# second-state/qwen3_asr_rs

Measured on NVIDIA H100. Metric: real-time factor (audio-sec/wall-sec) Qwen3-ASR-0.6B 30s clips, higher is better.
Workload: dtype f32 (bf16 weights, fp32-exact activations)

## Files before the change

qwen3_asr_rs_b200/csrc/decode_mega.cu:

```cuda
#include "mega_common.cuh"

namespace asrb {

namespace mega {

struct Params {
    const DecLayerW* layers;
    const bf16* lm_head;
    const bf16* embed;
    const float* final_norm;
    const float* rope_cos; const float* rope_sin;
    float eps;
    int L, H, QD, KVD, I, V, nq, nkv, group;
    float* x;
    float* kcache; float* vcache; size_t cache_layer_stride; int max_ctx;
    int nsplit;
    float* part_val; int* part_idx;
    int* pos; int* done; int* next_id; int* ids_out; int* n_out; int max_new;
    unsigned* bar;
    uint2* qkv_ll; uint2* part_ll; uint2* attn_ll; uint2* x_ll; uint2* act_ll;
    long long* dbg;
    int pf_ahead;
};

static constexpr int PF_AHEAD = 2;

template <int H, int QD, int I>
struct ChunkCursor {
    int l, ph, r; Slice s; bool done;
    const DecLayerW* ltab;
    __device__ void load(const Params& p) {
        if (l >= p.L) { if (l == p.L && ph == 0) s = make_slice(p.lm_head, p.V, H, 1); else { done = true; return; } }
        else {
            const DecLayerW w = ltab[l];
            s = ph == 0 ? make_slice(w.wqkv, QD + 2 * p.KVD, H, 1) : ph == 1 ? make_slice(w.wo, H, QD, 1)
              : ph == 2 ? make_slice(w.wgu, 2 * I, H, 2) : make_slice(w.wdown, H, I, 1);
        }
        r = s.r0;
    }
    __device__ void init(const Params& p, const DecLayerW* table) { ltab = table; l = 0; ph = 0; done = false; load(p); }
    __device__ bool next(const Params& p, const bf16*& src, uint32_t& bytes) {
        while (!done && r >= s.r1) {
            if (l >= p.L) { done = true; break; }
            if (++ph == 4) { ph = 0; ++l; }
            load(p);
        }
        if (done) return false;
        const int rows = min(s.rpc, s.r1 - r);
        src = s.W + (size_t)r * s.K; bytes = (uint32_t)rows * s.K * 2;
        r += s.rpc;
        return true;
    }
};

template <class Cursor>
__device__ __forceinline__ void produce(const Slice& s, const Ring& ring, uint32_t& q, Cursor& pf, const Params& p) {
    for (int r = s.r0; r < s.r1; r += s.rpc, ++q) {
        int rows = min(s.rpc, s.r1 - r);
        uint32_t slot = q % ring.nslot, par = (q / ring.nslot) & 1;
        mbar_wait(&ring.empty[slot], par ^ 1);
        uint32_t bytes = (uint32_t)rows * s.K * 2;
        mbar_expect_tx(&ring.full[slot], bytes);
        bulk_g2s(ring.slots + (size_t)slot * SLOT_BYTES, s.W + (size_t)r * s.K, bytes, &ring.full[slot]);
        const bf16* psrc; uint32_t pbytes;
        if (p.pf_ahead > 0 && pf.next(p, psrc, pbytes)) l2_prefetch(psrc, pbytes);
    }
}

template <int K>
__device__ __forceinline__ void load_xr(const float* xs, float (&xr)[K / 32], int lane) {
    const int sw = ((lane >> 2) & 1) * 4;
#pragma unroll
    for (int c = 0; c < K / 256; ++c) {
        const float4 a = *reinterpret_cast<const float4*>(xs + (c * 32 + lane) * 8 + sw);
        const float4 b = *reinterpret_cast<const float4*>(xs + (c * 32 + lane) * 8 + 4 - sw);
        xr[c * 8 + 0] = a.x; xr[c * 8 + 1] = a.y; xr[c * 8 + 2] = a.z; xr[c * 8 + 3] = a.w;
        xr[c * 8 + 4] = b.x; xr[c * 8 + 5] = b.y; xr[c * 8 + 6] = b.z; xr[c * 8 + 7] = b.w;
    }
}
template <int K>
__device__ __forceinline__ void load_xr_norm(const float* xs, const float* wn, float r, float (&xr)[K / 32], int lane) {
    const int sw = ((lane >> 2) & 1) * 4;
#pragma unroll
    for (int c = 0; c < K / 256; ++c) {
        const int o = (c * 32 + lane) * 8;
        const float4 a = *reinterpret_cast<const float4*>(xs + o + sw), b = *reinterpret_cast<const float4*>(xs + o + 4 - sw);
        const float4 wa = *reinterpret_cast<const float4*>(wn + o + sw), wb = *reinterpret_cast<const float4*>(wn + o + 4 - sw);
        xr[c * 8 + 0] = (a.x * r) * wa.x; xr[c * 8 + 1] = (a.y * r) * wa.y; xr[c * 8 + 2] = (a.z * r) * wa.z; xr[c * 8 + 3] = (a.w * r) * wa.w;
        xr[c * 8 + 4] = (b.x * r) * wb.x; xr[c * 8 + 5] = (b.y * r) * wb.y; xr[c * 8 + 6] = (b.z * r) * wb.z; xr[c * 8 + 7] = (b.w * r) * wb.w;
    }
}

template <int K>
__device__ __forceinline__ float row_dot(const uint4* wrow, const float (&xr)[K / 32], int lane) {
    float a0 = 0.f, a1 = 0.f;
#pragma unroll
    for (int c = 0; c < K / 256; ++c) {
        const uint4 w = wrow[c * 32 + lane];
        a0 = fmaf(bf16_lo(w.x), xr[c * 8 + 0], a0); a1 = fmaf(bf16_hi(w.x), xr[c * 8 + 1], a1);
        a0 = fmaf(bf16_lo(w.y), xr[c * 8 + 2], a0); a1 = fmaf(bf16_hi(w.y), xr[c * 8 + 3], a1);
        a0 = fmaf(bf16_lo(w.z), xr[c * 8 + 4], a0); a1 = fmaf(bf16_hi(w.z), xr[c * 8 + 5], a1);
        a0 = fmaf(bf16_lo(w.w), xr[c * 8 + 6], a0); a1 = fmaf(bf16_hi(w.w), xr[c * 8 + 7], a1);
    }
    return warp_sum(a0 + a1);
}
template <int K>
__device__ __forceinline__ float row_dot2(const uint4* w0, const uint4* w1, const float (&xr)[K / 32], int lane) {
    float a0 = 0.f, a1 = 0.f, b0 = 0.f, b1 = 0.f;
#pragma unroll
    for (int c = 0; c < K / 256; ++c) {
        const uint4 w = w0[c * 32 + lane], v = w1[c * 32 + lane];
        a0 = fmaf(bf16_lo(w.x), xr[c * 8 + 0], a0); a1 = fmaf(bf16_hi(w.x), xr[c * 8 + 1], a1);
        b0 = fmaf(bf16_lo(v.x), xr[c * 8 + 0], b0); b1 = fmaf(bf16_hi(v.x), xr[c * 8 + 1], b1);
        a0 = fmaf(bf16_lo(w.y), xr[c * 8 + 2], a0); a1 = fmaf(bf16_hi(w.y), xr[c * 8 + 3], a1);
        b0 = fmaf(bf16_lo(v.y), xr[c * 8 + 2], b0); b1 = fmaf(bf16_hi(v.y), xr[c * 8 + 3], b1);
        a0 = fmaf(bf16_lo(w.z), xr[c * 8 + 4], a0); a1 = fmaf(bf16_hi(w.z), xr[c * 8 + 5], a1);
        b0 = fmaf(bf16_lo(v.z), xr[c * 8 + 4], b0); b1 = fmaf(bf16_hi(v.z), xr[c * 8 + 5], b1);
        a0 = fmaf(bf16_lo(w.w), xr[c * 8 + 6], a0); a1 = fmaf(bf16_hi(w.w), xr[c * 8 + 7], a1);
        b0 = fmaf(bf16_lo(v.w), xr[c * 8 + 6], b0); b1 = fmaf(bf16_hi(v.w), xr[c * 8 + 7], b1);
    }
    const float ra = a0 + a1, rb = b0 + b1;
    const bool hi = lane & 16;
    float keep = (hi ? rb : ra) + __shfl_xor_sync(0xffffffffu, hi ? ra : rb, 16);
#pragma unroll
    for (int o = 8; o > 0; o >>= 1) keep += __shfl_xor_sync(0xffffffffu, keep, o);
    return keep;
}

template <int K>
__device__ __forceinline__ float row_dot_smem(const uint4* wrow, const float* xs, int lane) {
    float a0 = 0.f, a1 = 0.f;
    const int sw = ((lane >> 2) & 1) * 4;
#pragma unroll 4
    for (int c = 0; c < K / 256; ++c) {
        const uint4 w = wrow[c * 32 + lane];
        const float4 xa = *reinterpret_cast<const float4*>(xs + (c * 32 + lane) * 8 + sw);
        const float4 xb = *reinterpret_cast<const float4*>(xs + (c * 32 + lane) * 8 + 4 - sw);
        a0 = fmaf(bf16_lo(w.x), xa.x, a0); a1 = fmaf(bf16_hi(w.x), xa.y, a1);
        a0 = fmaf(bf16_lo(w.y), xa.z, a0); a1 = fmaf(bf16_hi(w.y), xa.w, a1);
        a0 = fmaf(bf16_lo(w.z), xb.x, a0); a1 = fmaf(bf16_hi(w.z), xb.y, a1);
        a0 = fmaf(bf16_lo(w.w), xb.z, a0); a1 = fmaf(bf16_hi(w.w), xb.w, a1);
    }
    return warp_sum(a0 + a1);
}


template <int K>
__device__ __forceinline__ float row_dot4(const uint4* w0, const uint4* w1, const uint4* w2, const uint4* w3,
                                          const float (&xr)[K / 32], int lane) {
    float a0 = 0.f, a1 = 0.f, b0 = 0.f, b1 = 0.f, c0 = 0.f, c1 = 0.f, d0 = 0.f, d1 = 0.f;
// ... 215 lines not shown
                    const bool two = ub + 1 < units_here;
                    v0 = row_dot2<KX>(base + (size_t)ub * (K / 8), base + (size_t)(two ? ub + 1 : ub) * (K / 8),
                                      reinterpret_cast<const float (&)[KX / 32]>(xr), lane);
                    act = ((lane & 15) == 0) && (sub == 0 || two);
                    row = r + ub + sub;
                } else {
                    if (XREG) v0 = row_dot<KX>(base + (size_t)ub * (K / 8), reinterpret_cast<const float (&)[KX / 32]>(xr), lane);
                    else v0 = row_dot_smem<K>(base + (size_t)ub * (K / 8), xs, lane);
                    act = lane == 0; row = r + ub;
                }
                if (EPI == ME_STORE) {
                    if (act) ll_store(out + row, v0, tag);
                } else if (EPI == ME_RESID) {
                    if (act) { const float nv = xres[row - s.r0] + v0; xres[row - s.r0] = nv; ll_store(out + row, nv, tag); }
                } else {
                    if (act && v0 > best_v) { best_v = v0; best_i = row; }
                }
            }
        }
        unit += (units_here + UPW - 1) / UPW * UPW;
        CF();
        __syncwarp();
        if (lane == 0) mbar_arrive(&ring.empty[slot]);
    }
    CF();
#undef CF
    if (!XREG) cons_sync();
}

__device__ __forceinline__ float norm_scale(float ss, int n, float eps, float* red) {
    const int tid = threadIdx.x;
    ss = warp_sum(ss);
    if ((tid & 31) == 0) red[tid >> 5] = ss;
    cons_sync();
    float tot = 0.f;
#pragma unroll
    for (int i = 0; i < NCONS_WARPS; ++i) tot += red[i];
    return 1.0f / sqrtf(tot / n + eps);
}

__device__ __forceinline__ void head_norm_rope(const uint2* __restrict__ src, uint32_t tag, const float* __restrict__ nw,
                                               float eps, const float* __restrict__ cs, const float* __restrict__ sn,
                                               float* dst, int lane) {
    float v[4];
    ll_poll4(src + lane, 32, tag, v);
    float ss = warp_sum(v[0] * v[0] + v[1] * v[1] + v[2] * v[2] + v[3] * v[3]);
    const float r = 1.0f / sqrtf(ss / 128.f + eps);
#pragma unroll
    for (int i = 0; i < 4; ++i) v[i] = (v[i] * r) * nw[lane + 32 * i];
#pragma unroll
    for (int i = 0; i < 2; ++i) {
        const int d = lane + 32 * i;
        const float c = cs[d], s = sn[d];
        const float a = v[i], b = v[i + 2];
        dst[d] = a * c - b * s;
        dst[d + 64] = b * c + a * s;
    }
}

#define MEGA_FINE(k)                                                                                    \
    do {                                                                                               \
        if (dbg_row && tid == 0 && l == 5) dbg_row[400 + (k)] = clock64();                              \
    } while (0)
#define MEGA_GT(k)                                                                                     \
    do {                                                                                               \
        if (p.dbg && tid == 0 && l == 5) {                                                             \
            unsigned long long t_; asm volatile("mov.u64 %0, %%globaltimer;" : "=l"(t_));               \
            p.dbg[512 + 3 * blockIdx.x + (k)] = (long long)t_;                                         \
        }                                                                                              \
    } while (0)
#define MEGA_MARK()                                                                                    \
    do {                                                                                               \
        if (dbg_row && tid == 0 && dbg_i < DBG_SLOTS) dbg_row[dbg_i++] = clock64();                    \
    } while (0)

template <int H, int QD, int I, int NS>
__global__ void __launch_bounds__(NTHREADS, 1) decode_step_kernel(const Params p) {
    constexpr int XS_FLOATS = (I > XS_MIN ? I : XS_MIN) + 64;
    extern __shared__ __align__(128) uint8_t smem[];
    constexpr int PARAM_FLOATS = 2 * H + 2 * HD;
    Ring ring;
    ring.slots = smem;
    ring.nslot = NS;
    uint8_t* kv_smem = smem + (size_t)NS * SLOT_BYTES;
    float* xs = reinterpret_cast<float*>(kv_smem + 2 * KV_TILE_BYTES);
    float* xres = xs + XS_FLOATS;
    float* pbuf = xres + XRES_MAX;
    float* ropes = pbuf + 2 * PARAM_FLOATS;
    DecLayerW* ltab = reinterpret_cast<DecLayerW*>(ropes + 128);
    uint64_t* bars = reinterpret_cast<uint64_t*>(ltab + MAX_LAYERS);
    ring.full = bars; ring.empty = bars + NSLOT_MAX;
    uint64_t* kv_full = bars + 2 * NSLOT_MAX; uint64_t* kv_empty = kv_full + 1;
    uint64_t* p_full = kv_empty + 1; uint64_t* p_empty = p_full + 2;
    float* red = reinterpret_cast<float*>(bars + 2 * NSLOT_MAX + 6);
    int* ired = reinterpret_cast<int*>(red + 64);
    float* part = reinterpret_cast<float*>(ired + 64);
    const int tid = threadIdx.x, lane = tid & 31, warp = tid >> 5;
    const bool is_producer = warp == NCONS_WARPS;

    if (__ldcg(p.done) != 0) return;

    if (tid == 0) {
        for (int i = 0; i < NS; ++i) { mbar_init(&ring.full[i], 1); mbar_init(&ring.empty[i], NCONS_WARPS); }
        mbar_init(kv_full, 1); mbar_init(kv_empty, NCONS_WARPS);
        for (int i = 0; i < 2; ++i) { mbar_init(&p_full[i], 1); mbar_init(&p_empty[i], NCONS_WARPS); }
        asm volatile("fence.mbarrier_init.release.cluster;" ::: "memory");
    }
    const int pos = __ldcg(p.pos);
    {
        const uint2* src = reinterpret_cast<const uint2*>(p.layers);
        uint2* dst = reinterpret_cast<uint2*>(ltab);
        for (int i = tid; i < p.L * (int)(sizeof(DecLayerW) / 8); i += NTHREADS) dst[i] = src[i];
        if (tid < 64) ropes[tid] = p.rope_cos[(size_t)pos * 64 + tid];
        else if (tid < 128) ropes[tid] = p.rope_sin[(size_t)pos * 64 + tid - 64];
    }
    __syncthreads();

    const bool att_cta = (int)blockIdx.x < p.nkv * p.nsplit;
    const int att_g = blockIdx.x / p.nsplit, att_sp = blockIdx.x % p.nsplit, att_j0 = att_sp * KV_KEYS;
    const int n_old = att_cta ? max(0, min(pos - att_j0, KV_KEYS)) : 0;
    uint32_t kvq = 0;
    uint32_t q = 0;
    if (is_producer) {
        if (lane == 0) {
            ChunkCursor<H, QD, I> pf;
            pf.init(p, ltab);
            {
                const bf16* psrc; uint32_t pbytes;
                for (int i = 0; i < p.pf_ahead; ++i) if (pf.next(p, psrc, pbytes)) l2_prefetch(psrc, pbytes);
            }
            const size_t kv_row = ((size_t)att_g * p.max_ctx + att_j0) * HD;
            if (n_old > 0) {
                l2_prefetch(p.kcache + kv_row, (uint32_t)n_old * HD * 4);
                l2_prefetch(p.vcache + kv_row, (uint32_t)n_old * HD * 4);
            }
            for (int l = 0; l <= p.L; ++l) {
                {
                    float* pb = pbuf + (l & 1) * PARAM_FLOATS;
                    mbar_wait(&p_empty[l & 1], ((l >> 1) & 1) ^ 1);
                    if (l < p.L) {
                        const DecLayerW w = ltab[l];
                        mbar_expect_tx(&p_full[l & 1], (uint32_t)(2 * H + 2 * HD) * 4);
                        bulk_g2s(pb, w.ln_in, H * 4, &p_full[l & 1]);
                        bulk_g2s(pb + H, w.ln_post, H * 4, &p_full[l & 1]);
                        bulk_g2s(pb + 2 * H, w.qnorm, HD * 4, &p_full[l & 1]);
                        bulk_g2s(pb + 2 * H + HD, w.knorm, HD * 4, &p_full[l & 1]);
                    } else {
                        mbar_expect_tx(&p_full[l & 1], (uint32_t)H * 4);
                        bulk_g2s(pb, p.final_norm, H * 4, &p_full[l & 1]);
                        break;
                    }
                }
                const DecLayerW w = ltab[l];
                produce(make_slice(w.wqkv, QD + 2 * p.KVD, H, 1), ring, q, pf, p);
                if (n_old > 0) {
                    const uint32_t bytes = (uint32_t)n_old * HD * 4;
                    if (l + 1 < p.L) {
                        l2_prefetch(p.kcache + (size_t)(l + 1) * p.cache_layer_stride + kv_row, bytes);
                        l2_prefetch(p.vcache + (size_t)(l + 1) * p.cache_layer_stride + kv_row, bytes);
                    }
                    mbar_wait(kv_empty, (kvq & 1) ^ 1);
                    mbar_expect_tx(kv_full, 2 * bytes);
                    const size_t off = (size_t)l * p.cache_layer_stride + kv_row;
                    bulk_g2s(kv_smem, p.kcache + off, bytes, kv_full);
                    bulk_g2s(kv_smem + KV_TILE_BYTES, p.vcache + off, bytes, kv_full);
                    ++kvq;
                }
                produce(make_slice(w.wo, H, QD, 1), ring, q, pf, p);
                produce(make_slice(w.wgu, 2 * I, H, 2), ring, q, pf, p);
                produce(make_slice(w.wdown, H, I, 1), ring, q, pf, p);
            }
            produce(make_slice(p.lm_head, p.V, H, 1), ring, q, pf, p);
            {
                ChunkCursor<H, QD, I> nx;
                nx.init(p, ltab);
                const bf16* psrc; uint32_t pbytes;
                for (int i = 0; i < p.pf_ahead; ++i) if (nx.next(p, psrc, pbytes)) l2_prefetch(psrc, pbytes);
            }
        }
        return;
    }

    long long* dbg_row = nullptr; int dbg_i = 0;
    if (p.dbg && (blockIdx.x == 0 || blockIdx.x == gridDim.x - 1)) dbg_row = p.dbg + (blockIdx.x == 0 ? 0 : DBG_SLOTS);
    MEGA_MARK();
    const int half = HD / 2;
    const float* cs = ropes;
    const float* sn = ropes + half;
    const unsigned G = gridDim.x;
    float best_v = -INFINITY; int best_i = 0x7fffffff;
    const unsigned epoch = __ldcg(p.bar + 1);
    const uint32_t tag_base = (epoch & 0xffffffu) << 8;
    const Slice xsl = make_slice(nullptr, H, QD, 1);
    Slice sl_qkv = make_slice(nullptr, QD + 2 * p.KVD, H, 1), sl_o = make_slice(nullptr, H, QD, 1),
          sl_gu = make_slice(nullptr, 2 * I, H, 2), sl_dn = make_slice(nullptr, H, I, 1);
    for (int i = tid; i < xsl.r1 - xsl.r0; i += NCONS) xres[i] = __ldcg(p.x + xsl.r0 + i);

    for (int l = 0; l < p.L; ++l) {
        const DecLayerW w = ltab[l];
        const uint32_t tl = tag_base | ((uint32_t)l << 3);
        const float* pb = pbuf + (l & 1) * PARAM_FLOATS;
        mbar_wait(&p_full[l & 1], (l >> 1) & 1);
        float nr;
        {
            float ss = 0.f;
            if (l == 0) { for (int i = tid; i < H; i += NCONS) { const float v = __ldcg(p.x + i); xs[xs_swz(i)] = v; ss = fmaf(v, v, ss); } }
            else { MEGA_FINE(0); MEGA_FINE(1); ss = ll_gather(p.x_ll, H, (tag_base | ((uint32_t)(l - 1) << 3)) | PH_XD, xs); MEGA_FINE(2); }
            nr = norm_scale(ss, H, p.eps, red);
            MEGA_FINE(3);
        }
        consume<H, ME_STORE>(sl_qkv, ring, q, xs, p.qkv_ll, tl | PH_QKV, xres, best_v, best_i, pb, nr);
        MEGA_FINE(4);
        MEGA_GT(0);
        MEGA_MARK();
        {
            const int nloc = n_old;
            const int nact = min(p.nsplit, (pos + KV_KEYS - 1) / KV_KEYS);
            const bool merger = att_cta && att_sp == 0;
            if (nloc > 0) {
                const int g = att_g;
                float* qs = xs;
                float* kn = qs + p.group * HD;
                float* vn = kn + HD;
                float* sc = vn + HD;
                float* ml = sc + p.group * KV_KEYS;
                float* osum = ml + 8;
                float* wml = osum + NCONS_WARPS * 2 * HD;
                float* snew = wml + NCONS_WARPS * 4;
                float* Ks = reinterpret_cast<float*>(kv_smem);
                float* Vs = reinterpret_cast<float*>(kv_smem + KV_TILE_BYTES);
                MEGA_FINE(24);
                cons_sync();
                if (warp < p.group) head_norm_rope(p.qkv_ll + (size_t)(g * p.group + warp) * HD, tl | PH_QKV, pb + 2 * H, p.eps, cs, sn, qs + warp * HD, lane);
                else if (warp == p.group && merger) head_norm_rope(p.qkv_ll + QD + (size_t)g * HD, tl | PH_QKV, pb + 2 * H + HD, p.eps, cs, sn, kn, lane);
                else if (warp == p.group + 1 && merger) {
                    float vv[4];
                    ll_poll4(p.qkv_ll + QD + p.KVD + (size_t)g * HD + lane, 32, tl | PH_QKV, vv);
#pragma unroll
                    for (int i = 0; i < 4; ++i) vn[lane + 32 * i] = vv[i];
                }
                MEGA_FINE(25);
                mbar_wait(kv_full, kvq & 1);
                cons_sync();
                MEGA_FINE(26);
                if (merger) {
                    if (tid < HD) {
                        float* kc = p.kcache + (size_t)l * p.cache_layer_stride + ((size_t)g * p.max_ctx + pos) * HD;
                        float* vc = p.vcache + (size_t)l * p.cache_layer_stride + ((size_t)g * p.max_ctx + pos) * HD;
                        kc[tid] = kn[tid]; vc[tid] = vn[tid];
                    }
                    if (warp >= NCONS_WARPS - p.group) {
                        const int hq = warp - (NCONS_WARPS - p.group);
                        const float4 a = *reinterpret_cast<const float4*>(qs + hq * HD + lane * 4);
                        const float4 b = *reinterpret_cast<const float4*>(kn + lane * 4);
                        const float sn_ = warp_sum(fmaf(a.x, b.x, fmaf(a.y, b.y, fmaf(a.z, b.z, a.w * b.w))));
                        if (lane == 0) snew[hq] = sn_ / sqrtf((float)HD);
                    }
                }
                MEGA_FINE(27);
                if (p.group == 2) {
                    const float4 q0 = *reinterpret_cast<const float4*>(qs + lane * 4);
                    const float4 q1 = *reinterpret_cast<const float4*>(qs + HD + lane * 4);
                    float pv[16];
#pragma unroll
                    for (int kk = 0; kk < 8; ++kk) {
                        const int j = warp + 8 * kk;
                        const float4 kv = *reinterpret_cast<const float4*>(Ks + j * HD + lane * 4);
                        pv[2 * kk] = fmaf(kv.x, q0.x, fmaf(kv.y, q0.y, fmaf(kv.z, q0.z, kv.w * q0.w)));
                        pv[2 * kk + 1] = fmaf(kv.x, q1.x, fmaf(kv.y, q1.y, fmaf(kv.z, q1.z, kv.w * q1.w)));
                    }
#pragma unroll
                    for (int o = 16, n = 16; n > 1; o >>= 1, n >>= 1) {
                        const bool up = lane & o;
#pragma unroll
                        for (int i = 0; i < n / 2; ++i) {
                            const float send = up ? pv[i] : pv[i + n / 2];
                            const float keep = up ? pv[i + n / 2] : pv[i];
                            pv[i] = keep + __shfl_xor_sync(0xffffffffu, send, o);
                        }
                    }
                    pv[0] += __shfl_xor_sync(0xffffffffu, pv[0], 1);
                    const bool mine = warp + 8 * (lane >> 2) < nloc;
                    const float sv = mine ? pv[0] / sqrtf((float)HD) : -INFINITY;
                    float mw = sv;
                    mw = fmaxf(mw, __shfl_xor_sync(0xffffffffu, mw, 4));
                    mw = fmaxf(mw, __shfl_xor_sync(0xffffffffu, mw, 8));
                    mw = fmaxf(mw, __shfl_xor_sync(0xffffffffu, mw, 16));
                    const float ev = mine ? expf(sv - mw) : 0.f;
                    float lw = ev;
                    lw += __shfl_xor_sync(0xffffffffu, lw, 4);
                    lw += __shfl_xor_sync(0xffffffffu, lw, 8);
                    lw += __shfl_xor_sync(0xffffffffu, lw, 16);
                    float4 o0 = make_float4(0.f, 0.f, 0.f, 0.f), o1 = o0;
#pragma unroll
                    for (int kk = 0; kk < 8; ++kk) {
                        const int j = warp + 8 * kk;
                        const float4 vv = *reinterpret_cast<const float4*>(Vs + j * HD + lane * 4);
                        const float e0 = __shfl_sync(0xffffffffu, ev, 4 * kk), e1 = __shfl_sync(0xffffffffu, ev, 4 * kk + 2);
                        if (j < nloc) {
                            o0.x = fmaf(e0, vv.x, o0.x); o0.y = fmaf(e0, vv.y, o0.y); o0.z = fmaf(e0, vv.z, o0.z); o0.w = fmaf(e0, vv.w, o0.w);
                            o1.x = fmaf(e1, vv.x, o1.x); o1.y = fmaf(e1, vv.y, o1.y); o1.z = fmaf(e1, vv.z, o1.z); o1.w = fmaf(e1, vv.w, o1.w);
                        }
                    }
                    *reinterpret_cast<float4*>(osum + (warp * 2 + 0) * HD + lane * 4) = o0;
                    *reinterpret_cast<float4*>(osum + (warp * 2 + 1) * HD + lane * 4) = o1;
                    if (lane == 0 || lane == 2) { wml[(warp * 2 + (lane >> 1)) * 2] = mw; wml[(warp * 2 + (lane >> 1)) * 2 + 1] = lw; }
                    cons_sync();
                    MEGA_FINE(28);
                    {
                        const int hq = tid / HD, d = tid - hq * HD;
                        float M = -INFINITY;
#pragma unroll
                        for (int w8 = 0; w8 < NCONS_WARPS; ++w8) M = fmaxf(M, wml[(w8 * 2 + hq) * 2]);
                        float acc = 0.f, Ls = 0.f;
#pragma unroll
                        for (int w8 = 0; w8 < NCONS_WARPS; ++w8) {
                            const float f = expf(wml[(w8 * 2 + hq) * 2] - M);
                            acc = fmaf(f, osum[(w8 * 2 + hq) * HD + d], acc);
                            Ls = fmaf(f, wml[(w8 * 2 + hq) * 2 + 1], Ls);
                        }
                        uint2* rec = p.part_ll + ((size_t)blockIdx.x * 2 + hq) * PSTRIDE;
                        ll_store(rec + d, acc, tl | PH_PART);
                        if (d < 2) ll_store(rec + HD + d, d == 0 ? M : Ls, tl | PH_PART);
                    }
                    MEGA_FINE(29);
                } else {
                    for (int idx = tid; idx < p.group * KV_KEYS; idx += NCONS) {
                        const int hq = idx / KV_KEYS, j = idx - hq * KV_KEYS;
                        if (j < nloc) {
                            const float* kr = Ks + j * HD; const float* qr = qs + hq * HD;
                            float a0 = 0.f, a1 = 0.f;
#pragma unroll 8
                            for (int dd = 0; dd < HD; dd += 2) {
                                const int d0 = (dd + j) & (HD - 1), d1 = (dd + 1 + j) & (HD - 1);
                                a0 = fmaf(kr[d0], qr[d0], a0); a1 = fmaf(kr[d1], qr[d1], a1);
                            }
                            sc[hq * KV_KEYS + j] = (a0 + a1) / sqrtf((float)HD);
                        }
                    }
                    cons_sync();
                    if (warp < p.group) {
                        float mx = -INFINITY;
                        for (int j = lane; j < nloc; j += 32) mx = fmaxf(mx, sc[warp * KV_KEYS + j]);
                        mx = warp_max(mx);
                        float sum = 0.f;
                        for (int j = lane; j < nloc; j += 32) {
                            float e = expf(sc[warp * KV_KEYS + j] - mx);
                            sc[warp * KV_KEYS + j] = e; sum += e;
                        }
                        sum = warp_sum(sum);
                        if (lane == 0) { ml[warp * 2] = mx; ml[warp * 2 + 1] = sum; }
                    }
                    cons_sync();
                    for (int idx = tid; idx < p.group * HD; idx += NCONS) {
                        const int hq = idx / HD, d = idx - hq * HD;
                        float acc = 0.f;
                        for (int j = 0; j < nloc; ++j) acc = fmaf(sc[hq * KV_KEYS + j], Vs[j * HD + d], acc);
                        uint2* rec = p.part_ll + ((size_t)blockIdx.x * p.group + hq) * PSTRIDE;
                        ll_store(rec + d, acc, tl | PH_PART);
                        if (d < 2) ll_store(rec + HD + d, ml[hq * 2 + d], tl | PH_PART);
                    }
                }
                {
                    asm volatile("fence.proxy.async.shared::cta;" ::: "memory");
                    __syncwarp();
                    if (lane == 0) mbar_arrive(kv_empty);
                    ++kvq;
                }
                MEGA_FINE(30);
                MEGA_GT(1);
                if (merger) {
                    for (int idx = tid; idx < p.group * HD; idx += NCONS) {
                        const int hq = idx / HD, d = idx - hq * HD;
                        const uint32_t tg = tl | PH_PART;
                        constexpr int RB = 9;
                        uint2 mv, lv, ov[RB];
                        bool ok;
                        auto load_round = [&](int u0) {
#pragma unroll
                            for (int u = 0; u < RB; ++u) {
                                if (u0 + u < nact) {
                                    const uint2* rec = p.part_ll + ((size_t)(g * p.nsplit + u0 + u) * p.group + hq) * PSTRIDE;
                                    asm volatile("ld.relaxed.gpu.global.v2.u32 {%0, %1}, [%2];" : "=r"(ov[u].x), "=r"(ov[u].y) : "l"(rec + d) : "memory");
                                }
                            }
                        };
                        auto round_ok = [&](int u0) {
                            bool k = true;
#pragma unroll
                            for (int u = 0; u < RB; ++u) if (u0 + u < nact) k = k && (ov[u].y == tg);
                            return k;
                        };
                        do {
                            mv.y = tg; lv.y = tg; mv.x = 0u; lv.x = 0u;
                            if (lane < nact) {
                                const uint2* rec = p.part_ll + ((size_t)(g * p.nsplit + lane) * p.group + hq) * PSTRIDE;
                                asm volatile("ld.relaxed.gpu.global.v2.u32 {%0, %1}, [%2];" : "=r"(mv.x), "=r"(mv.y) : "l"(rec + HD) : "memory");
                                asm volatile("ld.relaxed.gpu.global.v2.u32 {%0, %1}, [%2];" : "=r"(lv.x), "=r"(lv.y) : "l"(rec + HD + 1) : "memory");
                            }
                            load_round(0);
                            ok = __all_sync(0xffffffffu, (mv.y == tg) && (lv.y == tg) && round_ok(0));
                        } while (!ok);
                        MEGA_FINE(35);
                        const float m_l = lane < nact ? __uint_as_float(mv.x) : (lane == nact ? snew[hq] : -INFINITY);
                        const float l_l = lane < nact ? __uint_as_float(lv.x) : (lane == nact ? 1.f : 0.f);
                        const float M = warp_max(m_l);
                        const float f = expf(m_l - M);
                        const float Lsum = warp_sum(f * l_l);
                        float O = __shfl_sync(0xffffffffu, f, nact) * vn[d];
                        for (int u0 = 0; u0 < nact; u0 += RB) {
                            if (u0 > 0) { do { load_round(u0); ok = __all_sync(0xffffffffu, round_ok(u0)); } while (!ok); }
#pragma unroll
                            for (int u = 0; u < RB; ++u)
                                if (u0 + u < nact) O = fmaf(__shfl_sync(0xffffffffu, f, u0 + u), __uint_as_float(ov[u].x), O);
                        }
                        ll_store(p.attn_ll + (size_t)(g * p.group + hq) * HD + d, O / Lsum, tl | PH_ATTN);
                    }
                }
                MEGA_FINE(31);
                cons_sync();
            }
        }
        MEGA_MARK();
        MEGA_FINE(32);
        ll_gather(p.attn_ll, QD, tl | PH_ATTN, xs);
        MEGA_FINE(33);
        MEGA_GT(2);
        cons_sync();
        consume<QD, ME_RESID>(sl_o, ring, q, xs, p.x_ll, tl | PH_XO, xres, best_v, best_i, nullptr, 1.f, nullptr, part);
        MEGA_FINE(34);
        MEGA_MARK();
        cons_sync();
        {
            MEGA_FINE(8); MEGA_FINE(9);
            const float ss = ll_gather(p.x_ll, H, tl | PH_XO, xs); MEGA_FINE(10);
            nr = norm_scale(ss, H, p.eps, red); MEGA_FINE(11);
        }
        consume<H, ME_SWIGLU>(sl_gu, ring, q, xs, p.act_ll, tl | PH_ACT, xres, best_v, best_i, pb + H, nr, (dbg_row && l == 5) ? dbg_row + 440 : nullptr);
        MEGA_FINE(12);
        MEGA_FINE(13);
        MEGA_MARK();
        MEGA_FINE(16); MEGA_FINE(17);
        ll_gather(p.act_ll, I, tl | PH_ACT, xs); MEGA_FINE(18);
        cons_sync();
        consume<I, ME_RESID>(sl_dn, ring, q, xs, p.x_ll, tl | PH_XD, xres, best_v, best_i, nullptr, 1.f, nullptr, part);
        MEGA_FINE(19);
        MEGA_FINE(20);
        MEGA_MARK();
        cons_sync();
        if (lane == 0) mbar_arrive(&p_empty[l & 1]);
    }
    float nrf;
    {
        const float ss = ll_gather(p.x_ll, H, (tag_base | ((uint32_t)(p.L - 1) << 3)) | PH_XD, xs);
        mbar_wait(&p_full[p.L & 1], (p.L >> 1) & 1);
        nrf = norm_scale(ss, H, p.eps, red);
    }
    consume<H, ME_ARGMAX>(make_slice(p.lm_head, p.V, H, 1), ring, q, xs, nullptr, 0u, xres, best_v, best_i,
                          pbuf + (p.L & 1) * PARAM_FLOATS, nrf);
    MEGA_MARK();
#pragma unroll
    for (int o = 8; o <= 16; o <<= 1) {
        const float ov = __shfl_xor_sync(0xffffffffu, best_v, o); const int oi = __shfl_xor_sync(0xffffffffu, best_i, o);
        if (ov > best_v || (ov == best_v && oi < best_i)) { best_v = ov; best_i = oi; }
    }
    cons_sync();
    if (lane == 0) { red[warp] = best_v; ired[warp] = best_i; }
    cons_sync();
    int& is_last = ired[63];
    if (tid == 0) {
        float v = -INFINITY; int idx = 0x7fffffff;
        for (int wq = 0; wq < NCONS_WARPS; ++wq)
            if (red[wq] > v || (red[wq] == v && ired[wq] < idx)) { v = red[wq]; idx = ired[wq]; }
        p.part_val[blockIdx.x] = v; p.part_idx[blockIdx.x] = idx;
        __threadfence();
        unsigned t = atomicAdd(p.bar, 1u);
        is_last = (t == G - 1);
    }
    cons_sync();
    if (!is_last) return;
    __threadfence();
    {
        float v = -INFINITY; int idx = 0x7fffffff;
        for (int i = tid; i < (int)G; i += NCONS) {
            float pv = __ldcg(p.part_val + i); int pi = __ldcg(p.part_idx + i);
            if (pv > v || (pv == v && pi < idx)) { v = pv; idx = pi; }
        }
#pragma unroll
        for (int o = 16; o > 0; o >>= 1) {
            float ov = __shfl_xor_sync(0xffffffffu, v, o); int oi = __shfl_xor_sync(0xffffffffu, idx, o);
            if (ov > v || (ov == v && oi < idx)) { v = ov; idx = oi; }
        }
        if (lane == 0) { red[warp] = v; ired[warp] = idx; }
        cons_sync();
        int& tok_s = ired[62];
        if (tid == 0) {
            for (int wq = 1; wq < NCONS_WARPS; ++wq)
                if (red[wq] > v || (red[wq] == v && ired[wq] < idx)) { v = red[wq]; idx = ired[wq]; }
            int tok = idx;
            const int n = *p.n_out;
            if (tok == 151643 || tok == 151645 || n >= p.max_new) { *p.done = 1; *p.next_id = -1; tok = -1; }
            else { p.ids_out[n] = tok; *p.n_out = n + 1; *p.pos = pos + 1; *p.next_id = tok; }
            tok_s = tok;
            p.bar[0] = 0;
            p.bar[1] = p.bar[1] + 1;
        }
        cons_sync();
        const int tok = tok_s;
        if (tok >= 0) {
            const bf16* e = p.embed + (size_t)tok * H;
            for (int i = tid; i < H; i += NCONS) p.x[i] = __bfloat162float(e[i]);
        }
    }
}

}

static long long* g_last_dbg = nullptr;

static int mega_xs_floats(int I) { return std::max(I, mega::XS_MIN) + 64; }
static size_t mega_smem_bytes(int H, int I, int nslot) {
    return (size_t)nslot * mega::SLOT_BYTES + 2 * mega::KV_TILE_BYTES +
           (mega_xs_floats(I) + mega::XRES_MAX + 2 * (2 * H + 2 * mega::HD) + 128) * 4 + mega::MAX_LAYERS * sizeof(DecLayerW) +
           (2 * mega::NSLOT_MAX + 6) * 8 + 64 * 4 + 64 * 4 + 128 * 4 + 64;
}
static int mega_nslot(const asrb_dims& c) { return c.hidden_size > 1024 ? 3 : 4; }

template <int H, int QD, int I> static bool dims_match(const asrb_dims& c) {
    return c.hidden_size == H && c.num_attention_heads * c.head_dim == QD && c.intermediate_size == I;
}

bool decode_mega_supported(const Model& m, int B, int ctx) {
    const int max_ctx = ctx;
    const asrb_dims& c = m.d.c;
    if (B < 1 || c.head_dim != 128) return false;
    const int group = c.num_attention_heads / c.num_key_value_heads;
    if (group + 2 > mega::NCONS_WARPS) return false;
    if ((size_t)(group * 128 + 256 + group * mega::KV_KEYS + 8 + mega::NCONS_WARPS * 2 * 128 + mega::NCONS_WARPS * 4 + 8) > (size_t)mega_xs_floats(c.intermediate_size)) return false;
    if (m.ctx->smem_optin < mega_smem_bytes(c.hidden_size, c.intermediate_size, mega_nslot(c))) return false;
    if ((c.hidden_size + m.ctx->sm_count - 1) / m.ctx->sm_count + 1 > mega::XRES_MAX) return false;
    if (c.num_hidden_layers > 32) return false;
    if ((max_ctx + mega::KV_KEYS - 1) / mega::KV_KEYS > mega::MAX_SPLITS) return false;
    if (((max_ctx + mega::KV_KEYS - 1) / mega::KV_KEYS) * c.num_key_value_heads > m.ctx->sm_count) return false;
    return dims_match<1024, 2048, 3072>(c) || dims_match<2048, 2048, 6144>(c) || dims_match<256, 512, 512>(c);
}

size_t decode_mega_part_floats(const Model& m) {
    const asrb_dims& c = m.d.c;
    const int group = c.num_attention_heads / c.num_key_value_heads;
    const size_t words = (size_t)m.d.qkv_dim + (size_t)m.ctx->sm_count * group * mega::PSTRIDE + m.d.q_dim + c.hidden_size +
                         c.intermediate_size + 64;
    return 2 * words + 64;
}

void launch_decode_step_mega(const Model& m, const DecodeBufs& b, int B, float* kcache, float* vcache,
                             size_t cache_layer_stride, size_t cache_seq_stride, int max_ctx, int ctx_now, const MegaBufs& mb,
                             cudaStream_t st, int64_t* launches) {
    ASRB_REQUIRE(decode_mega_supported(m, B, ctx_now), ASRB_ERR_STATE, "fused decode step not supported for this model/batch/context");
    ASRB_REQUIRE(m.d_dec_layers && mb.bar && mb.part, ASRB_ERR_STATE, "fused decode step buffers missing");
    const asrb_dims& c = m.d.c;
    const int G = m.ctx->sm_count;
    const int group = c.num_attention_heads / c.num_key_value_heads;
    const int nsplit = std::min(mega::MAX_SPLITS, std::min(G / c.num_key_value_heads, (max_ctx + mega::KV_KEYS - 1) / mega::KV_KEYS));
    const size_t smem = mega_smem_bytes(c.hidden_size, c.intermediate_size, mega_nslot(c));
    const void* fn = nullptr;
    if (dims_match<1024, 2048, 3072>(c)) fn = (const void*)mega::decode_step_kernel<1024, 2048, 3072, 4>;
    else if (dims_match<2048, 2048, 6144>(c)) fn = (const void*)mega::decode_step_kernel<2048, 2048, 6144, 3>;
    else fn = (const void*)mega::decode_step_kernel<256, 512, 512, 4>;
    ASRB_CUDA_CHECK(cudaFuncSetAttribute(fn, cudaFuncAttributeMaxDynamicSharedMemorySize, (int)smem));
    for (int sb = 0; sb < B; ++sb) {
        mega::Params p{};
        p.layers = m.d_dec_layers; p.lm_head = m.lm_head; p.embed = m.embed; p.final_norm = m.final_norm_sw;
        p.rope_cos = m.rope_cos; p.rope_sin = m.rope_sin; p.eps = (float)c.rms_norm_eps;
        p.L = c.num_hidden_layers; p.H = c.hidden_size; p.QD = m.d.q_dim; p.KVD = m.d.kv_dim; p.I = c.intermediate_size;
        p.V = c.vocab_size; p.nq = c.num_attention_heads; p.nkv = c.num_key_value_heads; p.group = group;
        p.x = b.x + (size_t)sb * c.hidden_size;
        p.kcache = kcache + (size_t)sb * cache_seq_stride; p.vcache = vcache + (size_t)sb * cache_seq_stride;
        p.cache_layer_stride = cache_layer_stride; p.max_ctx = max_ctx; p.nsplit = nsplit;
        p.part_val = b.part_val; p.part_idx = b.part_idx;
        p.pos = b.pos + sb; p.done = b.done + sb; p.next_id = b.next_id + sb;
        p.ids_out = b.ids_out + (size_t)sb * b.max_new; p.n_out = b.n_out + sb; p.max_new = b.max_new;
        p.bar = mb.bar;
        uint2* w = reinterpret_cast<uint2*>(mb.part);
        p.qkv_ll = w; w += m.d.qkv_dim;
        p.part_ll = w; w += (size_t)G * group * mega::PSTRIDE;
        p.attn_ll = w; w += m.d.q_dim;
        p.x_ll = w; w += c.hidden_size;
        p.act_ll = w; w += c.intermediate_size;
        p.dbg = mb.dbg;
        g_last_dbg = mb.dbg;
        static const int pf_env = [] { const char* e = getenv("ASRB_MEGA_PF"); return e ? atoi(e) : mega::PF_AHEAD; }();
        p.pf_ahead = pf_env;
        if (mb.steps_issued && ++*mb.steps_issued >= 0xFFFF00u) {
            ASRB_CUDA_CHECK(cudaMemsetAsync(mb.part, 0, mb.part_bytes, st));
            const unsigned one = 1;
            ASRB_CUDA_CHECK(cudaMemcpyAsync(mb.bar + 1, &one, sizeof(one), cudaMemcpyHostToDevice, st));
            *mb.steps_issued = 1;
        }
        void* args[] = {(void*)&p};
        ASRB_CUDA_CHECK(cudaLaunchCooperativeKernel(fn, dim3(G), dim3(mega::NTHREADS), args, smem, st));
        if (launches) *launches += 1;
    }
}

int decode_mega_debug_timeline(long long* out, int cap) {
    if (!g_last_dbg || cap < 2 * mega::DBG_SLOTS) return 0;
    cudaDeviceSynchronize();
    cudaMemcpy(out, g_last_dbg, 2 * mega::DBG_SLOTS * sizeof(long long), cudaMemcpyDeviceToHost);
    return mega::DBG_SLOTS;
}
int decode_mega_dbg_slots() { return 4 * mega::DBG_SLOTS; }

}
```

qwen3_asr_rs_b200/csrc/mega_common.cuh:

```cuda
#pragma once
#include "internal.h"

namespace asrb {
namespace mega {

static constexpr int NCONS_WARPS = 8;
static constexpr int NCONS = NCONS_WARPS * 32;
static constexpr int NTHREADS = NCONS + 32;
static constexpr int SLOT_BYTES = 32 * 1024;
static constexpr int NSLOT_MAX = 4;
static constexpr int KV_KEYS = 64;
static constexpr int KV_TILE_BYTES = KV_KEYS * 128 * 4;
static constexpr int XS_MIN = 3072;
static constexpr int XRES_MAX = 64;
static constexpr int MAX_LAYERS = 32;
static constexpr int HD = 128;
static constexpr int PSTRIDE = HD + 2;
static constexpr int DBG_SLOTS = 1024;
static constexpr int MAX_SPLITS = 18;

enum { PH_QKV = 1, PH_PART = 2, PH_ATTN = 3, PH_XO = 4, PH_ACT = 5, PH_XD = 6 };

__device__ __forceinline__ uint32_t smem_u32(const void* p) { return (uint32_t)__cvta_generic_to_shared(p); }
__device__ __forceinline__ void mbar_init(uint64_t* bar, uint32_t count) {
    asm volatile("mbarrier.init.shared::cta.b64 [%0], %1;" ::"r"(smem_u32(bar)), "r"(count));
}
__device__ __forceinline__ void mbar_expect_tx(uint64_t* bar, uint32_t bytes) {
    asm volatile("mbarrier.arrive.expect_tx.shared::cta.b64 _, [%0], %1;" ::"r"(smem_u32(bar)), "r"(bytes) : "memory");
}
__device__ __forceinline__ void mbar_arrive(uint64_t* bar) {
    asm volatile("mbarrier.arrive.shared::cta.b64 _, [%0];" ::"r"(smem_u32(bar)) : "memory");
}
__device__ __forceinline__ void mbar_wait(uint64_t* bar, uint32_t parity) {
    asm volatile(
        "{\n"
        ".reg .pred p;\n"
        "WAIT_LOOP:\n"
        "mbarrier.try_wait.parity.shared::cta.b64 p, [%0], %1;\n"
        "@p bra.uni WAIT_DONE;\n"
        "bra.uni WAIT_LOOP;\n"
        "WAIT_DONE:\n"
        "}\n" ::"r"(smem_u32(bar)), "r"(parity) : "memory");
}
__device__ __forceinline__ void bulk_g2s(void* dst, const void* src, uint32_t bytes, uint64_t* bar) {
    asm volatile("cp.async.bulk.shared::cluster.global.mbarrier::complete_tx::bytes [%0], [%1], %2, [%3];"
                 ::"r"(smem_u32(dst)), "l"(src), "r"(bytes), "r"(smem_u32(bar)) : "memory");
}
__device__ __forceinline__ void cons_sync() { asm volatile("bar.sync 1, %0;" ::"n"(NCONS) : "memory"); }

__device__ __forceinline__ void ll_store(uint2* p, float v, uint32_t tag) {
    const unsigned long long val = ((unsigned long long)tag << 32) | (unsigned long long)__float_as_uint(v);
    asm volatile("red.relaxed.gpu.global.max.u64 [%0], %1;" ::"l"(p), "l"(val) : "memory");
}
__device__ __forceinline__ uint4 ll_load2(const uint2* p) {
    uint4 v;
    asm volatile("ld.relaxed.gpu.global.v4.u32 {%0, %1, %2, %3}, [%4];" : "=r"(v.x), "=r"(v.y), "=r"(v.z), "=r"(v.w) : "l"(p) : "memory");
    return v;
}
__device__ __forceinline__ float ll_poll1(const uint2* p, uint32_t tag) {
    uint2 v;
    do {
        asm volatile("ld.relaxed.gpu.global.v2.u32 {%0, %1}, [%2];" : "=r"(v.x), "=r"(v.y) : "l"(p) : "memory");
    } while (v.y != tag);
    return __uint_as_float(v.x);
}
__device__ __forceinline__ void ll_poll4(const uint2* p, int stride, uint32_t tag, float (&out)[4]) {
    uint2 v[4];
    bool ok;
    do {
#pragma unroll
        for (int i = 0; i < 4; ++i)
            asm volatile("ld.relaxed.gpu.global.v2.u32 {%0, %1}, [%2];" : "=r"(v[i].x), "=r"(v[i].y) : "l"(p + (size_t)i * stride) : "memory");
        ok = (v[0].y == tag) && (v[1].y == tag) && (v[2].y == tag) && (v[3].y == tag);
    } while (!ok);
#pragma unroll
    for (int i = 0; i < 4; ++i) out[i] = __uint_as_float(v[i].x);
}
__device__ __forceinline__ int xs_swz(int e) { const int k = e >> 2; return ((k ^ ((k >> 3) & 1)) << 2) | (e & 3); }
__device__ __forceinline__ float ll_gather(const uint2* buf, int n, uint32_t tag, float* xs) {
    float ss = 0.f;
    const int pairs = n >> 1;
    constexpr int U = 8;
    for (int i0 = threadIdx.x; i0 < pairs; i0 += U * NCONS) {
        uint4 v[U];
#pragma unroll
        for (int u = 0; u < U; ++u) v[u] = make_uint4(0u, 0u, 0u, 0u);
        bool ok;
        do {
            ok = true;
#pragma unroll
            for (int u = 0; u < U; ++u) {
                const int i = i0 + u * NCONS;
                if (i < pairs && !(v[u].y == tag && v[u].w == tag)) v[u] = ll_load2(buf + 2 * i);
            }
#pragma unroll
            for (int u = 0; u < U; ++u) {
                const int i = i0 + u * NCONS;
                if (i < pairs) ok = ok && (v[u].y == tag) && (v[u].w == tag);
            }
        } while (!ok);
#pragma unroll
        for (int u = 0; u < U; ++u) {
            const int i = i0 + u * NCONS;
            if (i < pairs) {
                const float a = __uint_as_float(v[u].x), b = __uint_as_float(v[u].z);
                *reinterpret_cast<float2*>(xs + xs_swz(2 * i)) = make_float2(a, b);
                ss = fmaf(a, a, ss); ss = fmaf(b, b, ss);
            }
        }
    }
    return ss;
}

struct Ring {
    uint8_t* slots; uint64_t* full; uint64_t* empty;
    uint32_t nslot;
};

struct Slice { const bf16* W; int K, r0, r1, rpc; };
__device__ __forceinline__ Slice make_slice(const bf16* W, int N, int K, int rstep) {
    Slice s; s.W = W; s.K = K;
    const unsigned units = (unsigned)(N / rstep);
    const int u0 = (int)((blockIdx.x * units) / gridDim.x), u1 = (int)(((blockIdx.x + 1) * units) / gridDim.x);
    s.r0 = u0 * rstep; s.r1 = u1 * rstep;
    s.rpc = SLOT_BYTES / (K * 2);
    s.rpc &= ~1;
    return s;
}

__device__ __forceinline__ void l2_prefetch(const void* src, uint32_t bytes) {
    asm volatile("cp.async.bulk.prefetch.L2.global [%0], %1;" ::"l"(src), "r"(bytes) : "memory");
}

}
}
```

Baseline: 281.0.

## Route KV tiles through the weight ring, drop L2 prefetch, use evict-first hints

Removes the separate double-buffered KV tile buffer and its barriers. K and V tiles are now issued as ordinary slots in the weight TMA ring, and the freed shared memory deepens the ring from 4 to 6 slots (3 to 5 for the larger model). The L2 prefetch cursor, the ASRB_MEGA_PF knob and the KV L2 prefetches are removed, and weight loads now carry an L2 evict-first cache policy. This trades explicit cross-stage L2 prefetching for a deeper in-flight TMA pipeline. The risk is that KV tiles now serialize behind weight chunks in the ring order, and that evict-first may push out reusable data.

```diff
diff --git a/qwen3_asr_rs_b200/csrc/decode_mega.cu b/qwen3_asr_rs_b200/csrc/decode_mega.cu
--- a/qwen3_asr_rs_b200/csrc/decode_mega.cu
+++ b/qwen3_asr_rs_b200/csrc/decode_mega.cu
@@ -20,52 +20,9 @@
     unsigned* bar;
     uint2* qkv_ll; uint2* part_ll; uint2* attn_ll; uint2* x_ll; uint2* act_ll;
     long long* dbg;
-    int pf_ahead;
 };
 
-static constexpr int PF_AHEAD = 2;
-
-template <int H, int QD, int I>
-struct ChunkCursor {
-    int l, ph, r; Slice s; bool done;
-    const DecLayerW* ltab;
-    __device__ void load(const Params& p) {
-        if (l >= p.L) { if (l == p.L && ph == 0) s = make_slice(p.lm_head, p.V, H, 1); else { done = true; return; } }
-        else {
-            const DecLayerW w = ltab[l];
-            s = ph == 0 ? make_slice(w.wqkv, QD + 2 * p.KVD, H, 1) : ph == 1 ? make_slice(w.wo, H, QD, 1)
-              : ph == 2 ? make_slice(w.wgu, 2 * I, H, 2) : make_slice(w.wdown, H, I, 1);
-        }
-        r = s.r0;
-    }
-    __device__ void init(const Params& p, const DecLayerW* table) { ltab = table; l = 0; ph = 0; done = false; load(p); }
-    __device__ bool next(const Params& p, const bf16*& src, uint32_t& bytes) {
-        while (!done && r >= s.r1) {
-            if (l >= p.L) { done = true; break; }
-            if (++ph == 4) { ph = 0; ++l; }
-            load(p);
-        }
-        if (done) return false;
-        const int rows = min(s.rpc, s.r1 - r);
-        src = s.W + (size_t)r * s.K; bytes = (uint32_t)rows * s.K * 2;
-        r += s.rpc;
-        return true;
-    }
-};
-
-template <class Cursor>
-__device__ __forceinline__ void produce(const Slice& s, const Ring& ring, uint32_t& q, Cursor& pf, const Params& p) {
-    for (int r = s.r0; r < s.r1; r += s.rpc, ++q) {
-        int rows = min(s.rpc, s.r1 - r);
-        uint32_t slot = q % ring.nslot, par = (q / ring.nslot) & 1;
-        mbar_wait(&ring.empty[slot], par ^ 1);
-        uint32_t bytes = (uint32_t)rows * s.K * 2;
-        mbar_expect_tx(&ring.full[slot], bytes);
-        bulk_g2s(ring.slots + (size_t)slot * SLOT_BYTES, s.W + (size_t)r * s.K, bytes, &ring.full[slot]);
-        const bf16* psrc; uint32_t pbytes;
-        if (p.pf_ahead > 0 && pf.next(p, psrc, pbytes)) l2_prefetch(psrc, pbytes);
-    }
-}
+static_assert(KV_KEYS * HD * 4 == SLOT_BYTES, "K / V tiles travel through the weight ring: one tile per slot");
 
 template <int K>
 __device__ __forceinline__ void load_xr(const float* xs, float (&xr)[K / 32], int lane) {
@@ -447,17 +404,15 @@
     Ring ring;
     ring.slots = smem;
     ring.nslot = NS;
-    uint8_t* kv_smem = smem + (size_t)NS * SLOT_BYTES;
-    float* xs = reinterpret_cast<float*>(kv_smem + 2 * KV_TILE_BYTES);
+    float* xs = reinterpret_cast<float*>(smem + (size_t)NS * SLOT_BYTES);
     float* xres = xs + XS_FLOATS;
     float* pbuf = xres + XRES_MAX;
     float* ropes = pbuf + 2 * PARAM_FLOATS;
     DecLayerW* ltab = reinterpret_cast<DecLayerW*>(ropes + 128);
     uint64_t* bars = reinterpret_cast<uint64_t*>(ltab + MAX_LAYERS);
     ring.full = bars; ring.empty = bars + NSLOT_MAX;
-    uint64_t* kv_full = bars + 2 * NSLOT_MAX; uint64_t* kv_empty = kv_full + 1;
-    uint64_t* p_full = kv_empty + 1; uint64_t* p_empty = p_full + 2;
-    float* red = reinterpret_cast<float*>(bars + 2 * NSLOT_MAX + 6);
+    uint64_t* p_full = bars + 2 * NSLOT_MAX; uint64_t* p_empty = p_full + 2;
+    float* red = reinterpret_cast<float*>(bars + 2 * NSLOT_MAX + 4);
     int* ired = reinterpret_cast<int*>(red + 64);
     float* part = reinterpret_cast<float*>(ired + 64);
     const int tid = threadIdx.x, lane = tid & 31, warp = tid >> 5;
@@ -467,7 +422,6 @@
 
     if (tid == 0) {
         for (int i = 0; i < NS; ++i) { mbar_init(&ring.full[i], 1); mbar_init(&ring.empty[i], NCONS_WARPS); }
-        mbar_init(kv_full, 1); mbar_init(kv_empty, NCONS_WARPS);
         for (int i = 0; i < 2; ++i) { mbar_init(&p_full[i], 1); mbar_init(&p_empty[i], NCONS_WARPS); }
         asm volatile("fence.mbarrier_init.release.cluster;" ::: "memory");
     }
@@ -484,21 +438,21 @@
     const bool att_cta = (int)blockIdx.x < p.nkv * p.nsplit;
     const int att_g = blockIdx.x / p.nsplit, att_sp = blockIdx.x % p.nsplit, att_j0 = att_sp * KV_KEYS;
     const int n_old = att_cta ? max(0, min(pos - att_j0, KV_KEYS)) : 0;
-    uint32_t kvq = 0;
     uint32_t q = 0;
     if (is_producer) {
         if (lane == 0) {
-            ChunkCursor<H, QD, I> pf;
-            pf.init(p, ltab);
-            {
-                const bf16* psrc; uint32_t pbytes;
-                for (int i = 0; i < p.pf_ahead; ++i) if (pf.next(p, psrc, pbytes)) l2_prefetch(psrc, pbytes);
-            }
+            const uint64_t pol = l2_evict_first_policy();
+            auto issue = [&](const void* src, uint32_t bytes) __attribute__((always_inline)) {
+                const uint32_t slot = q % NS, par = (q / NS) & 1;
+                mbar_wait(&ring.empty[slot], par ^ 1);
+                mbar_expect_tx(&ring.full[slot], bytes);
+                bulk_g2s_hint(ring.slots + (size_t)slot * SLOT_BYTES, src, bytes, &ring.full[slot], pol);
+                ++q;
+            };
+            auto issue_slice = [&](const Slice& s) __attribute__((always_inline)) {
+                for (int r = s.r0; r < s.r1; r += s.rpc) issue(s.W + (size_t)r * s.K, (uint32_t)min(s.rpc, s.r1 - r) * s.K * 2);
+            };
             const size_t kv_row = ((size_t)att_g * p.max_ctx + att_j0) * HD;
-            if (n_old > 0) {
-                l2_prefetch(p.kcache + kv_row, (uint32_t)n_old * HD * 4);
-                l2_prefetch(p.vcache + kv_row, (uint32_t)n_old * HD * 4);
-            }
             for (int l = 0; l <= p.L; ++l) {
                 {
                     float* pb = pbuf + (l & 1) * PARAM_FLOATS;
@@ -517,31 +471,17 @@
                     }
                 }
                 const DecLayerW w = ltab[l];
-                produce(make_slice(w.wqkv, QD + 2 * p.KVD, H, 1), ring, q, pf, p);
+                issue_slice(make_slice(w.wqkv, QD + 2 * p.KVD, H, 1));
                 if (n_old > 0) {
-                    const uint32_t bytes = (uint32_t)n_old * HD * 4;
-                    if (l + 1 < p.L) {
-                        l2_prefetch(p.kcache + (size_t)(l + 1) * p.cache_layer_stride + kv_row, bytes);
-                        l2_prefetch(p.vcache + (size_t)(l + 1) * p.cache_layer_stride + kv_row, bytes);
-                    }
-                    mbar_wait(kv_empty, (kvq & 1) ^ 1);
-                    mbar_expect_tx(kv_full, 2 * bytes);
                     const size_t off = (size_t)l * p.cache_layer_stride + kv_row;
-                    bulk_g2s(kv_smem, p.kcache + off, bytes, kv_full);
-                    bulk_g2s(kv_smem + KV_TILE_BYTES, p.vcache + off, bytes, kv_full);
-                    ++kvq;
-                }
-                produce(make_slice(w.wo, H, QD, 1), ring, q, pf, p);
-                produce(make_slice(w.wgu, 2 * I, H, 2), ring, q, pf, p);
-                produce(make_slice(w.wdown, H, I, 1), ring, q, pf, p);
+                    issue(p.kcache + off, (uint32_t)n_old * HD * 4);
+                    issue(p.vcache + off, (uint32_t)n_old * HD * 4);
+                }
+                issue_slice(make_slice(w.wo, H, QD, 1));
+                issue_slice(make_slice(w.wgu, 2 * I, H, 2));
+                issue_slice(make_slice(w.wdown, H, I, 1));
             }
-            produce(make_slice(p.lm_head, p.V, H, 1), ring, q, pf, p);
-            {
-                ChunkCursor<H, QD, I> nx;
-                nx.init(p, ltab);
-                const bf16* psrc; uint32_t pbytes;
-                for (int i = 0; i < p.pf_ahead; ++i) if (nx.next(p, psrc, pbytes)) l2_prefetch(psrc, pbytes);
-            }
+            issue_slice(make_slice(p.lm_head, p.V, H, 1));
         }
         return;
     }
@@ -592,8 +532,9 @@
                 float* osum = ml + 8;
                 float* wml = osum + NCONS_WARPS * 2 * HD;
                 float* snew = wml + NCONS_WARPS * 4;
-                float* Ks = reinterpret_cast<float*>(kv_smem);
-                float* Vs = reinterpret_cast<float*>(kv_smem + KV_TILE_BYTES);
+                const uint32_t ksl = q % ring.nslot, vsl = (q + 1) % ring.nslot;
+                const float* Ks = reinterpret_cast<const float*>(ring.slots + (size_t)ksl * SLOT_BYTES);
+                const float* Vs = reinterpret_cast<const float*>(ring.slots + (size_t)vsl * SLOT_BYTES);
                 MEGA_FINE(24);
                 cons_sync();
                 if (warp < p.group) head_norm_rope(p.qkv_ll + (size_t)(g * p.group + warp) * HD, tl | PH_QKV, pb + 2 * H, p.eps, cs, sn, qs + warp * HD, lane);
@@ -605,7 +546,8 @@
                     for (int i = 0; i < 4; ++i) vn[lane + 32 * i] = vv[i];
                 }
                 MEGA_FINE(25);
-                mbar_wait(kv_full, kvq & 1);
+                mbar_wait(&ring.full[ksl], (q / ring.nslot) & 1);
+                mbar_wait(&ring.full[vsl], ((q + 1) / ring.nslot) & 1);
                 cons_sync();
                 MEGA_FINE(26);
                 if (merger) {
@@ -729,8 +671,8 @@
                 {
                     asm volatile("fence.proxy.async.shared::cta;" ::: "memory");
                     __syncwarp();
-                    if (lane == 0) mbar_arrive(kv_empty);
-                    ++kvq;
+                    if (lane == 0) { mbar_arrive(&ring.empty[ksl]); mbar_arrive(&ring.empty[vsl]); }
+                    q += 2;
                 }
                 MEGA_FINE(30);
                 MEGA_GT(1);
@@ -885,11 +827,11 @@
 
 static int mega_xs_floats(int I) { return std::max(I, mega::XS_MIN) + 64; }
 static size_t mega_smem_bytes(int H, int I, int nslot) {
-    return (size_t)nslot * mega::SLOT_BYTES + 2 * mega::KV_TILE_BYTES +
+    return (size_t)nslot * mega::SLOT_BYTES +
            (mega_xs_floats(I) + mega::XRES_MAX + 2 * (2 * H + 2 * mega::HD) + 128) * 4 + mega::MAX_LAYERS * sizeof(DecLayerW) +
-           (2 * mega::NSLOT_MAX + 6) * 8 + 64 * 4 + 64 * 4 + 128 * 4 + 64;
-}
-static int mega_nslot(const asrb_dims& c) { return c.hidden_size > 1024 ? 3 : 4; }
+           (2 * mega::NSLOT_MAX + 4) * 8 + 64 * 4 + 64 * 4 + 128 * 4 + 64;
+}
+static int mega_nslot(const asrb_dims& c) { return c.hidden_size > 1024 ? 5 : 6; }
 
 template <int H, int QD, int I> static bool dims_match(const asrb_dims& c) {
     return c.hidden_size == H && c.num_attention_heads * c.head_dim == QD && c.intermediate_size == I;
@@ -929,9 +871,9 @@
     const int nsplit = std::min(mega::MAX_SPLITS, std::min(G / c.num_key_value_heads, (max_ctx + mega::KV_KEYS - 1) / mega::KV_KEYS));
     const size_t smem = mega_smem_bytes(c.hidden_size, c.intermediate_size, mega_nslot(c));
     const void* fn = nullptr;
-    if (dims_match<1024, 2048, 3072>(c)) fn = (const void*)mega::decode_step_kernel<1024, 2048, 3072, 4>;
-    else if (dims_match<2048, 2048, 6144>(c)) fn = (const void*)mega::decode_step_kernel<2048, 2048, 6144, 3>;
-    else fn = (const void*)mega::decode_step_kernel<256, 512, 512, 4>;
+    if (dims_match<1024, 2048, 3072>(c)) fn = (const void*)mega::decode_step_kernel<1024, 2048, 3072, 6>;
+    else if (dims_match<2048, 2048, 6144>(c)) fn = (const void*)mega::decode_step_kernel<2048, 2048, 6144, 5>;
+    else fn = (const void*)mega::decode_step_kernel<256, 512, 512, 6>;
     ASRB_CUDA_CHECK(cudaFuncSetAttribute(fn, cudaFuncAttributeMaxDynamicSharedMemorySize, (int)smem));
     for (int sb = 0; sb < B; ++sb) {
         mega::Params p{};
@@ -954,8 +896,6 @@
         p.act_ll = w; w += c.intermediate_size;
         p.dbg = mb.dbg;
         g_last_dbg = mb.dbg;
-        static const int pf_env = [] { const char* e = getenv("ASRB_MEGA_PF"); return e ? atoi(e) : mega::PF_AHEAD; }();
-        p.pf_ahead = pf_env;
         if (mb.steps_issued && ++*mb.steps_issued >= 0xFFFF00u) {
             ASRB_CUDA_CHECK(cudaMemsetAsync(mb.part, 0, mb.part_bytes, st));
             const unsigned one = 1;
diff --git a/qwen3_asr_rs_b200/csrc/mega_common.cuh b/qwen3_asr_rs_b200/csrc/mega_common.cuh
--- a/qwen3_asr_rs_b200/csrc/mega_common.cuh
+++ b/qwen3_asr_rs_b200/csrc/mega_common.cuh
@@ -8,9 +8,8 @@
 static constexpr int NCONS = NCONS_WARPS * 32;
 static constexpr int NTHREADS = NCONS + 32;
 static constexpr int SLOT_BYTES = 32 * 1024;
-static constexpr int NSLOT_MAX = 4;
+static constexpr int NSLOT_MAX = 6;
 static constexpr int KV_KEYS = 64;
-static constexpr int KV_TILE_BYTES = KV_KEYS * 128 * 4;
 static constexpr int XS_MIN = 3072;
 static constexpr int XRES_MAX = 64;
 static constexpr int MAX_LAYERS = 32;
@@ -45,6 +44,15 @@
 __device__ __forceinline__ void bulk_g2s(void* dst, const void* src, uint32_t bytes, uint64_t* bar) {
     asm volatile("cp.async.bulk.shared::cluster.global.mbarrier::complete_tx::bytes [%0], [%1], %2, [%3];"
                  ::"r"(smem_u32(dst)), "l"(src), "r"(bytes), "r"(smem_u32(bar)) : "memory");
+}
+__device__ __forceinline__ uint64_t l2_evict_first_policy() {
+    uint64_t pol;
+    asm volatile("createpolicy.fractional.L2::evict_first.b64 %0, 1.0;" : "=l"(pol));
+    return pol;
+}
+__device__ __forceinline__ void bulk_g2s_hint(void* dst, const void* src, uint32_t bytes, uint64_t* bar, uint64_t pol) {
+    asm volatile("cp.async.bulk.shared::cluster.global.mbarrier::complete_tx::bytes.L2::cache_hint [%0], [%1], %2, [%3], %4;"
+                 ::"r"(smem_u32(dst)), "l"(src), "r"(bytes), "r"(smem_u32(bar)), "l"(pol) : "memory");
 }
 __device__ __forceinline__ void cons_sync() { asm volatile("bar.sync 1, %0;" ::"n"(NCONS) : "memory"); }
 
@@ -128,9 +136,5 @@
     return s;
 }
 
-__device__ __forceinline__ void l2_prefetch(const void* src, uint32_t bytes) {
-    asm volatile("cp.async.bulk.prefetch.L2.global [%0], %1;" ::"l"(src), "r"(bytes) : "memory");
-}
-
 }
 }
```

Result: faster. 295.4 (median of 6 runs) (+5.1%).
